# scttfrdmn/bwa-mem2-arm

Measured on AMD Instinct MI355X. Metric: M seed-extensions/sec (150 bp, band=100) at 1/2/4/8 MI355X vs CPU, higher is better.
Workload: dtype int16; 1 GPU; C2: 1000000 SeqPairs/GPU resident in HBM, 150 bp query / 300 bp ref, band w=100, cell_bits=16, h0 U[19,100]; pairs_per_gpu=1000000, parallelism=shard1 (independent pairs), distinct_gpus=1

## Files before the change

### bwa-mem2-arm_amd/csrc/bsw_pc.hip

```cpp
#include <hip/hip_runtime.h>
#include <stdint.h>
#include <stdlib.h>
#include <limits.h>
#include <utility>
#include "bsw_kernels.h"
#include "bsw_wave.h"

namespace bsw {

constexpr int kPcChunkDw = 17;
#ifndef BSW_PC_EXP_HALFHEAD
#define BSW_PC_EXP_HALFHEAD 0
#endif
#ifdef BSW_PC_STATS
__device__ unsigned long long g_pc_stats[13];
constexpr int kPcTimesMax = 1 << 16;
__device__ unsigned long long g_pc_times[kPcTimesMax][4];
#endif

struct PcRow {
    uint64_t enter;
    uint64_t fast;
    uint64_t left;
};

__device__ __forceinline__ uint64_t gbits(int lo, int n)
{
    uint64_t m;
    asm("s_bfm_b64 %0, %1, %2" : "=s"(m)
        : "s"(__builtin_amdgcn_readfirstlane(min(n, 63))), "s"(__builtin_amdgcn_readfirstlane(lo)));
    return m;
}

__device__ __forceinline__ uint32_t pack2(int v) { return ((uint32_t)v & 0xffffu) * 0x10001u; }

#define PC_SDWA(op, d, a, b, sel) \
    op "_sdwa " d ", " a ", " b " dst_sel:DWORD dst_unused:UNUSED_PAD src0_sel:DWORD src1_sel:" sel "\n\t"

#define PC_PH1_(X, EOUT, ESUB)                                                          \
    "v_pk_min_i16 %[s" X "], %[s" X "], %[h" X "]\n\t"                                      \
    "v_pk_add_u16 %[s" X "], %[s" X "], %[h" X "]\n\t"                                      \
    "v_pk_sub_i16 %[t" X "], %[s" X "], %[oe2]\n\t"                                         \
    "v_pk_max_i16 %[s" X "], %[s" X "], %[e" X "]\n\t"                                      \
    ESUB                                                                                     \
    "v_pk_max_i16 " EOUT ", " EOUT ", %[t" X "]\n\t"
#define PC_PH1(X, EOUT) PC_PH1_(X, EOUT, "v_pk_sub_i16 " EOUT ", %[e" X "], %[ed2]\n\t")
#define PC_PH1B(X, EOUT) PC_PH1_(X, EOUT, "v_pk_sub_u16 " EOUT ", %[e" X "], %[ed2] clamp\n\t")

#define PC_SCORES                                                                        \
    "v_perm_b32 %[y], %[phi], %[plo], %[q]\n\t"                                              \
    "v_pk_lshlrev_b16 %[sa], 8, %[y] op_sel_hi:[0,1]\n\t"                                    \
    "v_pk_ashrrev_i16 %[sa], 8, %[sa] op_sel_hi:[0,1]\n\t"                                   \
    "v_pk_ashrrev_i16 %[sb], 8, %[y] op_sel_hi:[0,1]\n\t"

#define PC_CELL(C, X, W)                                                                 \
    PC_SDWA("v_max_i32", C, "%[f]", "sext(%[s" X "])", W)                                    \
    "v_subrev_u32_e64 %[f], %[ed], %[f] clamp\n\t"                                           \
    PC_SDWA("v_max_i32", "%[f]", "%[f]", "sext(%[t" X "])", W)

#define PC_RESET(HP, RJ)                                                                 \
    "v_cmp_ne_u32_e32 vcc, " RJ ", %[begv]\n\t"                                              \
    "v_cndmask_b32_e32 " HP ", 0, " HP ", vcc\n\t"                                           \
    "v_cndmask_b32_e32 %[f], 0, %[f], vcc\n\t"
#define PC_MCELL(C, HP, X, W, J)                                                         \
    PC_CELL(C, X, W)                                                                         \
    "v_cmp_lt_i32_e32 vcc, " J ", %[endv]\n\t"                                               \
    "v_cndmask_b32_e32 " C ", " HP ", " C ", vcc\n\t"

#define PC_MWRITE(X, KEYSRC, LEFT)                                                       \
    "v_pk_sub_i16 %[y], %[jj" X "], %[endw]\n\t"                                             \
    "v_pk_ashrrev_i16 %[y], 15, %[y] op_sel_hi:[0,1]\n\t"                                    \
    "v_bfi_b32 %[h" X "], %[y], %[p" X "], %[h" X "]\n\t"                                    \
    "v_bfi_b32 %[e" X "], %[y], 0, %[e" X "]\n\t"                                            \
    KEYSRC                                                                                   \
    "v_and_b32_e32 %[p" X "], %[p" X "], %[y]\n\t"                                           \
    "v_pk_sub_i16 %[y], %[jj" X "], %[endm1w]\n\t"                                           \
    "v_pk_ashrrev_i16 %[y], 15, %[y] op_sel_hi:[0,1]\n\t"                                    \
    "v_bfi_b32 %[e" X "], %[y], %[x" X "], %[e" X "]\n\t"                                    \
    LEFT                                                                                     \
    "v_pk_max_u16 %[key], %[key], %[p" X "]\n\t"
#define PC_LEFTMASK(X)                                                                   \
    "v_pk_sub_i16 %[y], %[begm2w], %[jj" X "]\n\t"                                           \
    "v_pk_ashrrev_i16 %[y], 15, %[y] op_sel_hi:[0,1]\n\t"                                    \
    "v_and_b32_e32 %[p" X "], %[p" X "], %[y]\n\t"

#define PC_MASKED(CH0, CH1, CH2, CH3, KA, KB, LA, LB) PC_MASKED_(PC_PH1, CH0, CH1, CH2, CH3, KA, KB, LA, LB)
#define PC_MASKED_(PH, CH0, CH1, CH2, CH3, KA, KB, LA, LB)                               \
    PH("a", "%[xa]") PH("b", "%[xb]")                                                        \
    CH0 CH1                                                                                  \
    "v_lshl_or_b32 %[pa], %[c0], 16, %[h1]\n\t"                                              \
    CH2 CH3                                                                                  \
    "v_lshl_or_b32 %[pb], %[c2], 16, %[c1]\n\t"                                              \
    PC_MWRITE("a", KA, LA) PC_MWRITE("b", KB, LB)

#ifdef BSW_PC_STATS
#define PC_CNT(k) "v_add_u32_e32 %[ct" #k "], 1, %[ct" #k "]\n\t"
#define PC_CNT_OPS , [ct0] "+v"(ctr[0]), [ct1] "+v"(ctr[1]), [ct2] "+v"(ctr[2]), [ct3] "+v"(ctr[3])
#else
#define PC_CNT(k)
#define PC_CNT_OPS
#endif

#define PC_FAST_CHAIN                                                                    \
    PC_FAST_CHAIN_("v_alignbyte_b32 %[ha], %[pa], %[h1], 2\n\t", "v_alignbyte_b32 %[hb], %[h1], %[pa], 2\n\t")
#define PC_FAST_CHAIN_(A1, A2) PC_FAST_CHAIN__(A1, A2, "%[h1]")
#define PC_FAST_CHAIN__(A1, A2, H1O)                                                     \
    "v_pk_sub_u16 %[fp], %[f], %[e0e] op_sel_hi:[0,1] clamp\n\t"                            \
    "v_pk_max_i16 %[fp], %[fp], %[ta] op_sel_hi:[1,0]\n\t"                                  \
    "v_pk_max_i16 %[pa], %[fp], %[sa]\n\t"                                                  \
    "v_pk_sub_u16 %[fp], %[fp], %[ee2] op_sel:[1,0] clamp\n\t"                              \
    "v_pk_sub_i16 %[y], %[ta], %[e0e] op_sel:[1,0]\n\t"                                     \
    "v_pk_max_i16 %[fp], %[fp], %[y]\n\t"                                                   \
    A1                                                                                       \
    "v_pk_max_i16 %[fp], %[fp], %[tb] op_sel_hi:[1,0]\n\t"                                  \
    "v_pk_max_i16 " H1O ", %[fp], %[sb]\n\t"                                                \
    "v_sub_u32_sdwa %[f], %[fp], %[ed] clamp dst_sel:DWORD dst_unused:UNUSED_PAD src0_sel:WORD_1 src1_sel:DWORD\n\t" \
    A2                                                                                       \
    PC_SDWA("v_max_i32", "%[f]", "%[f]", "sext(%[tb])", "WORD_1")

#ifndef BSW_PC_RIGHT_EDGE
#define BSW_PC_RIGHT_EDGE 1
#endif
#define PC_REDGE(PH, KA, KB)                                                             \
    PH("a", "%[xa]") PH("b", "%[xb]")                                                        \
    PC_FAST_CHAIN__("v_alignbyte_b32 %[c0], %[pa], %[h1], 2\n\t",                            \
                    "v_alignbyte_b32 %[pb], %[c1], %[pa], 2\n\t", "%[c1]")                   \
    KA KB                                                                                    \
    "v_pk_sub_i16 %[sa], %[jja], %[endw]\n\t"                                                \
    "v_pk_sub_i16 %[sb], %[jjb], %[endw]\n\t"                                                \
    "v_pk_sub_i16 %[tb], %[jjb], %[endm1w]\n\t"                                              \
    "v_pk_ashrrev_i16 %[sa], 15, %[sa] op_sel_hi:[0,1]\n\t"                                  \
    "v_pk_ashrrev_i16 %[sb], 15, %[sb] op_sel_hi:[0,1]\n\t"                                  \
    "v_pk_ashrrev_i16 %[tb], 15, %[tb] op_sel_hi:[0,1]\n\t"                                  \
    "v_alignbyte_b32 %[ta], %[sb], %[sa], 2\n\t"                                             \
    "v_bfi_b32 %[h1], %[sa], %[c0], %[h1]\n\t"                                               \
    "v_bfi_b32 %[ha], %[sa], %[c0], %[ha]\n\t"                                               \
    "v_and_b32_e32 %[xa], %[xa], %[ta]\n\t"                                                  \
    "v_bfi_b32 %[h1], %[ta], %[pa], %[h1]\n\t"                                               \
    "v_bfi_b32 %[ea], %[sa], %[xa], %[ea]\n\t"                                               \
    "v_and_b32_e32 %[fp], %[fp], %[sa]\n\t"                                                  \
    "v_bfi_b32 %[h1], %[sb], %[pb], %[h1]\n\t"                                               \
    "v_bfi_b32 %[hb], %[sb], %[pb], %[hb]\n\t"                                               \
    "v_and_b32_e32 %[xb], %[xb], %[tb]\n\t"                                                  \
    "v_bfi_b32 %[h1], %[tb], %[c1], %[h1]\n\t"                                               \
    "v_bfi_b32 %[eb], %[sb], %[xb], %[eb]\n\t"                                               \
    "v_and_b32_e32 %[c2], %[c2], %[sb]\n\t"                                                  \
    "v_pk_max_u16 %[key], %[key], %[fp]\n\t"                                                 \
    "v_pk_max_u16 %[key], %[key], %[c2]\n\t"
#if BSW_PC_RIGHT_EDGE
#define PC_RBODY(PH, KA_M, KB_M, KA_R, KB_R) PC_REDGE(PH, KA_R, KB_R)
#else
#define PC_RBODY(PH, KA_M, KB_M, KA_R, KB_R)                                             \
    "v_lshrrev_b32_e32 %[h1], 16, %[h1]\n\t"                                                 \
    PC_MASKED_(PH, PC_MCELL("%[c0]", "%[h1]", "a", "WORD_0", "%[j0]"),                       \
                   PC_MCELL("%[c1]", "%[c0]", "a", "WORD_1", "%[j1]"),                       \
                   PC_MCELL("%[c2]", "%[c1]", "b", "WORD_0", "%[j2]"),                       \
                   PC_MCELL("%[h1]", "%[c2]", "b", "WORD_1", "%[j3]"), KA_M, KB_M, "", "")   \
    "v_lshlrev_b32_e32 %[h1], 16, %[h1]\n\t"
#endif
#define PC_LBODY(PH, KA_M, KB_M)                                                         \
    "v_lshrrev_b32_e32 %[h1], 16, %[h1]\n\t"          \
    PC_MASKED_(PH, PC_RESET("%[h1]", "%[r0]") PC_MCELL("%[c0]", "%[h1]", "a", "WORD_0", "%[j0]"), \
                   PC_RESET("%[c0]", "%[j1]") PC_MCELL("%[c1]", "%[c0]", "a", "WORD_1", "%[j1]"), \
                   PC_RESET("%[c1]", "%[j2]") PC_MCELL("%[c2]", "%[c1]", "b", "WORD_0", "%[j2]"), \
                   PC_RESET("%[c2]", "%[j3]") PC_MCELL("%[h1]", "%[c2]", "b", "WORD_1", "%[j3]"), \
                   KA_M, KB_M, PC_LEFTMASK("a"), PC_LEFTMASK("b"))                           \
    "v_lshlrev_b32_e32 %[h1], 16, %[h1]\n\t"

// ... 221 lines not shown
constexpr int kPcSeg = BSW_PC_SEG;
template <int QMAX> constexpr int pc_seg_len() { return QMAX <= 64 ? QMAX / 4 : kPcSeg; }
template <int QMAX, bool BY, int S, int... K>
__device__ __forceinline__ void pc_seg(std::integer_sequence<int, K...>, uint32_t (&hh)[(BY ? QMAX / 4 : QMAX / 2)],
                                       uint32_t (&ee)[(BY ? QMAX / 4 : QMAX / 2)], const uint32_t (&qs)[QMAX / 4], uint32_t plo,
                                       uint32_t phi, int &f, int &h1, uint32_t &key, uint32_t oe2, uint32_t ed2,
                                       int ed, const PcRow &r, uint32_t endw, uint32_t endm1w, uint32_t begm2w,
                                       int endv, int begv, const PcbSel &bs, uint32_t (&ctr)[4])
{
    constexpr int kSeg = sizeof...(K);
    constexpr uint64_t kSegMask = ((1ull << kSeg) - 1) << (kSeg * S);
    if (kSeg == QMAX / 4 || (r.enter & kSegMask))
        (pc_group_if<QMAX, BY, kSeg * S + K>(hh, ee, qs, plo, phi, f, h1, key, oe2, ed2, ed, r, endw, endm1w,
                                               begm2w, endv, begv, bs, ctr), ...);
}

template <int QMAX, bool BY, int... S>
__device__ __forceinline__ void pc_row(std::integer_sequence<int, S...>, uint32_t (&hh)[(BY ? QMAX / 4 : QMAX / 2)],
                                       uint32_t (&ee)[(BY ? QMAX / 4 : QMAX / 2)], const uint32_t (&qs)[QMAX / 4],
                                       uint32_t plo, uint32_t phi, int &f, int &h1, uint32_t &key,
                                       uint32_t oe2, uint32_t ed2, int ed, const PcRow &r,
                                       uint32_t endw, uint32_t endm1w, uint32_t begm2w, int endv,
                                       int begv, const PcbSel &bs, uint32_t (&ctr)[4])
{
    (pc_seg<QMAX, BY, S>(std::make_integer_sequence<int, pc_seg_len<QMAX>()>{}, hh, ee, qs, plo, phi, f, h1, key, oe2,
                         ed2, ed, r, endw, endm1w, begm2w, endv, begv, bs, ctr), ...);
}

template <int K>
__device__ __forceinline__ void pc_lastpos_reg(uint32_t hv, uint32_t endp1w, uint32_t &lp)
{
    constexpr uint32_t SC = (uint32_t)(2 * K) | ((uint32_t)(2 * K + 1) << 16);
    uint32_t c, m;
    asm volatile(
        "v_pk_min_u16 %[c], %[h], 1 op_sel_hi:[1,0]\n\t"
        "v_pk_mul_lo_u16 %[c], %[c], %[sc]\n\t"
        "v_pk_sub_i16 %[m], %[sc], %[e1]\n\t"
        "v_pk_ashrrev_i16 %[m], 15, %[m] op_sel_hi:[0,1]\n\t"
        "v_and_b32_e32 %[c], %[c], %[m]\n\t"
        "v_pk_max_u16 %[lp], %[lp], %[c]\n\t"
        : [lp] "+v"(lp), [c] "=&v"(c), [m] "=&v"(m)
        : [h] "v"(hv), [sc] "s"(SC), [e1] "v"(endp1w));
}

template <int QMAX, bool BY, int GG>
__device__ __forceinline__ bool pc_lastpos_group(const uint32_t (&hh)[(BY ? QMAX / 4 : QMAX / 2)], uint32_t endp1w,
                                                 bool pending, uint32_t &lp, int gstart)
{
    if (GG > gstart) return pending;
    if (__ballot(pending) == 0) return false;
    if constexpr (BY) {
        pc_lastpos_reg<2 * GG + 1>(__builtin_amdgcn_perm(hh[GG], hh[GG], kSelHi), endp1w, lp);
        pc_lastpos_reg<2 * GG>(__builtin_amdgcn_perm(hh[GG], hh[GG], kSelLo), endp1w, lp);
    } else {
        if constexpr (2 * GG + 1 < QMAX / 2) pc_lastpos_reg<2 * GG + 1>(hh[2 * GG + 1], endp1w, lp);
        pc_lastpos_reg<2 * GG>(hh[2 * GG], endp1w, lp);
    }
    return pending & (lp == 0u);
}

template <int QMAX, bool BY, int... G>
__device__ __forceinline__ int pc_lastpos(std::integer_sequence<int, G...>, const uint32_t (&hh)[(BY ? QMAX / 4 : QMAX / 2)],
                                          int end, bool need, int gstart)
{
    bool pending = need;
    uint32_t lp = 0;
    const uint32_t endp1w = pack2(end + 1);
    ((pending = pc_lastpos_group<QMAX, BY, QMAX / 4 - 1 - G>(hh, endp1w, pending, lp, gstart)), ...);
    return (int)max(lp & 0xffffu, lp >> 16);
}

#ifndef BSW_PC_EARLY_STOP
#define BSW_PC_EARLY_STOP 1
#endif
#ifndef BSW_PC_EARLY_SCAN
#define BSW_PC_EARLY_SCAN 1
#endif
#ifndef BSW_PC_SCAN_PHASE
#define BSW_PC_SCAN_PHASE 3
#endif

template <int K>
__device__ __forceinline__ void pc_ub_reg(uint32_t hv, uint32_t qw, uint32_t begw, uint32_t &ub)
{
    constexpr uint32_t SC = (uint32_t)(2 * K) | ((uint32_t)(2 * K + 1) << 16);
    uint32_t c, m;
    asm volatile(
        "v_pk_sub_i16 %[c], %[qw], %[sc]\n\t"
        "v_pk_ashrrev_i16 %[m], 15, %[c] op_sel_hi:[0,1]\n\t"
        "v_pk_add_u16 %[c], %[c], %[h]\n\t"
        "v_bfi_b32 %[c], %[m], 0, %[c]\n\t"
        "v_pk_sub_i16 %[m], %[bg], %[sc]\n\t"
        "v_pk_ashrrev_i16 %[m], 15, %[m] op_sel_hi:[0,1]\n\t"
        "v_and_b32_e32 %[c], %[c], %[m]\n\t"
        "v_pk_max_u16 %[ub], %[ub], %[c]\n\t"
        : [ub] "+v"(ub), [c] "=&v"(c), [m] "=&v"(m)
        : [h] "v"(hv), [qw] "v"(qw), [sc] "s"(SC), [bg] "v"(begw));
}

template <int QMAX, bool BY, int GG>
__device__ __forceinline__ void pc_ub_group(const uint32_t (&hh)[(BY ? QMAX / 4 : QMAX / 2)], uint32_t qw,
                                            uint32_t begw, uint32_t &ub, uint64_t enter)
{
    if (!((enter >> GG) & 1)) return;
    if constexpr (BY) {
        pc_ub_reg<2 * GG + 1>(__builtin_amdgcn_perm(hh[GG], hh[GG], kSelHi), qw, begw, ub);
        pc_ub_reg<2 * GG>(__builtin_amdgcn_perm(hh[GG], hh[GG], kSelLo), qw, begw, ub);
    } else {
        pc_ub_reg<2 * GG + 1>(hh[2 * GG + 1], qw, begw, ub);
        pc_ub_reg<2 * GG>(hh[2 * GG], qw, begw, ub);
    }
}

template <int QMAX, bool BY, int... G>
__device__ __forceinline__ int pc_ubscan(std::integer_sequence<int, G...>, const uint32_t (&hh)[(BY ? QMAX / 4 : QMAX / 2)],
                                         int qlen, int beg, uint64_t enter)
{
    uint32_t ub = 0;
    const uint32_t qw = pack2(qlen), begw = pack2(beg);
    (pc_ub_group<QMAX, BY, QMAX / 4 - 1 - G>(hh, qw, begw, ub, enter), ...);
    return (int)max(ub & 0xffffu, ub >> 16);
}

#ifndef BSW_PC_LEFT_SKIP
#define BSW_PC_LEFT_SKIP 1
#endif
#ifndef BSW_PC_SKIP_MASK
#define BSW_PC_SKIP_MASK 3
#endif
#ifndef BSW_PC_SKIP_ROW
#define BSW_PC_SKIP_ROW 1
#endif
#ifndef BSW_PC_SKIP_QMIN
#define BSW_PC_SKIP_QMIN 96
#endif
template <int QMAX> constexpr bool pc_left_skip() { return BSW_PC_LEFT_SKIP && QMAX >= BSW_PC_SKIP_QMIN; }

#ifndef BSW_PC_LEFT_PRUNE
#define BSW_PC_LEFT_PRUNE 1
#endif
#ifndef BSW_PC_PRUNE_QMIN
#define BSW_PC_PRUNE_QMIN 128
#endif
template <int QMAX, bool BY> constexpr bool pc_left_prune()
{
    return BSW_PC_LEFT_PRUNE && !BY && pc_left_skip<QMAX>() && QMAX >= BSW_PC_PRUNE_QMIN;
}
#ifndef BSW_PC_PRUNE_BRANCH
#define BSW_PC_PRUNE_BRANCH 1
#endif
constexpr int kPcPruned = 1 << 8;
template <bool PRUNE> __device__ __forceinline__ int pc_gz_of(int gz) { return PRUNE ? (gz & (kPcPruned - 1)) : gz; }

template <int K>
__device__ __forceinline__ void pc_pb_reg(uint32_t v, uint32_t gw, uint32_t bw, uint32_t &ub)
{
    constexpr uint32_t SC = (uint32_t)(2 * K) | ((uint32_t)(2 * K + 1) << 16);
    uint32_t c, m;
    asm volatile(
        "v_pk_sub_i16 %[c], %[gw], %[sc]\n\t"
        "v_pk_min_u16 %[m], %[v], 1 op_sel_hi:[1,0]\n\t"
        "v_pk_mul_lo_u16 %[c], %[c], %[m]\n\t"
        "v_pk_add_u16 %[c], %[c], %[v]\n\t"
        "v_pk_sub_i16 %[m], %[bw], %[sc]\n\t"
        "v_pk_ashrrev_i16 %[m], 15, %[m] op_sel_hi:[0,1]\n\t"
        "v_and_b32_e32 %[c], %[c], %[m]\n\t"
        "v_pk_max_u16 %[ub], %[ub], %[c]\n\t"
        : [ub] "+v"(ub), [c] "=&v"(c), [m] "=&v"(m)
        : [v] "v"(v), [gw] "v"(gw), [sc] "s"(SC), [bw] "v"(bw));
}

__device__ __forceinline__ uint32_t pc_pos2(uint32_t e)
{
    uint32_t r;
    asm volatile("v_pk_max_i16 %0, %1, 0" : "=v"(r) : "v"(e));
    return r;
}

struct PcPrune {
    bool pre;
    int qlen, beg, gsc;
    uint32_t npr;
};

template <int QMAX, bool BY, bool PRUNE, int G>
__device__ __forceinline__ void pc_gz_group(uint32_t (&hh)[(BY ? QMAX / 4 : QMAX / 2)],
                                            uint32_t (&ee)[(BY ? QMAX / 4 : QMAX / 2)], bool live, int &gz, PcPrune &pp)
{
    if constexpr (G < QMAX / 4) {
        if (pc_gz_of<PRUNE>(gz) != G) return;
        uint32_t z;
        if constexpr (BY) {
            asm volatile("v_or_b32_e32 %0, %1, %2" : "=v"(z) : "v"(hh[G]), "v"(ee[G]));
        } else {
            uint32_t t;
            asm volatile("v_pk_max_i16 %0, %2, 0\n\t"
                         "v_pk_max_i16 %1, %3, 0\n\t"
                         "v_or3_b32 %0, %0, %1, %4\n\t"
                         "v_or_b32_e32 %0, %0, %5"
                         : "=&v"(z), "=&v"(t)
                         : "v"(ee[2 * G]), "v"(ee[2 * G + 1]), "v"(hh[2 * G]), "v"(hh[2 * G + 1]));
        }
        if (__ballot(live && z != 0u) == 0) {
            gz = PRUNE ? gz + 1 : G + 1;
        } else if constexpr (PRUNE) {
            if (!pp.pre) return;
            uint32_t ub = 0;
            const uint32_t qw = pack2(pp.qlen), qm1w = pack2(pp.qlen - 1);
            const uint32_t bgw = pack2(pp.beg), bgm1w = pack2(pp.beg - 1);
            static_assert(!BY, "the byte planes are compiled without the prune");
            pc_pb_reg<2 * G + 1>(hh[2 * G + 1], qw, bgw, ub);
            pc_pb_reg<2 * G>(hh[2 * G], qw, bgw, ub);
            pc_pb_reg<2 * G + 1>(pc_pos2(ee[2 * G + 1]), qm1w, bgm1w, ub);
            pc_pb_reg<2 * G>(pc_pos2(ee[2 * G]), qm1w, bgm1w, ub);
            const int u = (int)max(ub & 0xffffu, ub >> 16);
            if (__ballot(live && u >= pp.gsc) == 0) {
                hh[2 * G] = 0u; hh[2 * G + 1] = 0u; ee[2 * G] = 0u; ee[2 * G + 1] = 0u;
                gz = (G + 1) | kPcPruned;
#ifdef BSW_PC_STATS
                pp.npr += 1;
#endif
            }
        }
    }
}

template <int QMAX, bool BY, bool PRUNE, int S, int... K>
__device__ __forceinline__ void pc_gz_seg(std::integer_sequence<int, K...>, uint32_t (&hh)[(BY ? QMAX / 4 : QMAX / 2)],
                                          uint32_t (&ee)[(BY ? QMAX / 4 : QMAX / 2)], bool live, int &gz, PcPrune &pp)
{
    if ((pc_gz_of<PRUNE>(gz) >> 3) != S) return;
    (pc_gz_group<QMAX, BY, PRUNE, 8 * S + K>(hh, ee, live, gz, pp), ...);
}

template <int QMAX, bool BY, bool PRUNE, int... S>
__device__ __forceinline__ void pc_gz_refresh(std::integer_sequence<int, S...>, uint32_t (&hh)[(BY ? QMAX / 4 : QMAX / 2)],
                                              uint32_t (&ee)[(BY ? QMAX / 4 : QMAX / 2)], bool live, int &gz, PcPrune &pp)
{
    (pc_gz_seg<QMAX, BY, PRUNE, S>(std::make_integer_sequence<int, 8>{}, hh, ee, live, gz, pp), ...);
}

template <int QMAX, int WPB, bool BY, bool REDO>
__global__ __launch_bounds__(64 * WPB, BY ? 3 : 2) void pc_kernel(const KParams kp, const int32_t w,
                                                    SeqPair *__restrict__ pairs,
                                                    const int32_t *__restrict__ order,
                                                    const int32_t n_in,
                                                    const uint8_t *__restrict__ ref,
                                                    const uint8_t *__restrict__ qer,
                                                    int32_t *__restrict__ err,
                                                    int32_t *__restrict__ redo,
                                                    int32_t *__restrict__ rcnt)
{
    constexpr bool PRUNE = !REDO && pc_left_prune<QMAX, BY>();
    constexpr int NG = QMAX / 4;
    constexpr int CDW = kPcChunkDw;
#ifdef BSW_PC_STATS
    const unsigned long long t_wave0 = wall_clock64();
#endif
    __shared__ uint32_t s_tgt[WPB][2][CDW][64];
    __shared__ uint2 s_prof[8];
    int32_t n = n_in;
    if constexpr (REDO) {
        n = min(n, *rcnt);
        if ((int)(blockIdx.x * blockDim.x) >= n) return;
    }
    if (threadIdx.x < 8) s_prof[threadIdx.x] = make_uint2(kp.prof[threadIdx.x][0], kp.prof[threadIdx.x][1]);
    __syncthreads();
    const int gid = blockIdx.x * blockDim.x + threadIdx.x;
    bool valid = gid < n;
    const int idx = valid ? (order ? order[gid] : gid) : 0;
    SeqPair *sp = pairs + idx;
    int idr = 0, idq = 0, tlen = 0, qlen = 0, h0 = 0;
    if (valid) {
        idr = sp->idr; idq = sp->idq; tlen = sp->len1; qlen = sp->len2; h0 = sp->h0;
        if (qlen >= QMAX || qlen < 0 || tlen < 0 || h0 < 0 || h0 + min(qlen, tlen) > 255 || idr < 0 || idq < 0) {
            atomicOr(err, 1);
            valid = false;
        }
    }
    uint32_t qs[NG];
    {
        uint32_t wv[NG + 1];
        const uintptr_t qa = (uintptr_t)(qer + idq);
        const uint32_t *wp = (const uint32_t *)(qa & ~(uintptr_t)3);
        const int sh = (int)(qa & 3);
        const int nw = (valid && qlen > 0) ? (sh + qlen + 3) >> 2 : 0;
        if (nw > 0) {
#pragma unroll
            for (int g = 0; g <= NG; ++g) wv[g] = wp[min(g, nw - 1)];
        } else {
#pragma unroll
            for (int g = 0; g <= NG; ++g) wv[g] = 0;
        }
#pragma unroll
        for (int g = 0; g < NG; ++g) {
            const uint32_t c = __builtin_amdgcn_alignbyte(wv[g + 1], wv[g], sh);
            qs[g] = __builtin_amdgcn_perm(c, c, 0x03010200u);
        }
    }
    constexpr int NP = (BY ? QMAX / 4 : QMAX / 2);
    uint32_t hh[NP], ee[NP];
    {
        const int oe_ins = kp.o_ins + kp.e_ins;
        if constexpr (BY) {
            __builtin_amdgcn_sched_barrier(0);
#pragma unroll
            for (int k = 0; k < NP; ++k) {
                uint32_t v[4];
#pragma unroll
                for (int t = 0; t < 4; ++t) {
                    const int j = 4 * k + t;
                    v[t] = (j == 0) ? (uint32_t)h0 : (j <= qlen) ? (uint32_t)max(h0 - oe_ins - (j - 1) * kp.e_ins, 0) : 0u;
                }
                hh[k] = v[0] | (v[1] << 8) | (v[2] << 16) | (v[3] << 24);
                asm volatile("" : "+v"(hh[k]));
                ee[k] = 0u;
            }
        } else {
#pragma unroll
            for (int k = 0; k < NP; ++k) {
                const int j0 = 2 * k, j1 = 2 * k + 1;
                const uint32_t a = (j0 == 0) ? (uint32_t)h0
                                 : (j0 <= qlen) ? (uint32_t)max(h0 - oe_ins - (j0 - 1) * kp.e_ins, 0) : 0u;
                const uint32_t b = (j1 <= qlen) ? (uint32_t)max(h0 - oe_ins - (j1 - 1) * kp.e_ins, 0) : 0u;
                hh[k] = a | (b << 16);
                ee[k] = 0u;
            }
        }
    }
    int wl = w;
    {
        const int ni = qlen * kp.maxsc + kp.end_bonus - kp.o_ins;
        const int nd = qlen * kp.maxsc + kp.end_bonus - kp.o_del;
        wl = min(wl, max((ni + kp.e_ins) / kp.e_ins, 1));
        wl = min(wl, max((nd + kp.e_del) / kp.e_del, 1));
    }
    int best = h0, best_i = -1, best_j = -1, max_ie = -1, gsc = -1, moff = 0, endc = qlen;
    bool alive = valid && tlen > 0;
    if (!valid) sp = nullptr;
    asm volatile("" : "+v"(sp));
    const uint8_t *tp = ref + idr;
    const int tsh = (int)((uintptr_t)tp & 3);
    const uint32_t *twp = (const uint32_t *)(tp - tsh);
    const int tlast = max((tsh + tlen - 1) >> 2, 0);
    const int wv = threadIdx.x >> 6, ln = threadIdx.x & 63;
    auto issue_chunk = [&](int ch) {
        uint32_t *dst = &s_tgt[wv][ch & 1][0][0];
#pragma unroll
        for (int k = 0; k < CDW; ++k)
            __builtin_amdgcn_global_load_lds((gptr_t)(twp + min(16 * ch + k, tlast)),
                                             (lptr_t)(dst + 64 * k), 4, 0, 0);
    };
    if (alive) { issue_chunk(0); issue_chunk(1); }
    uint32_t tcur = 0;
    const int wl_max = wave_max(alive ? wl : -1);
    const int wl_min = wave_min(alive ? wl : INT_MAX);
    const uint32_t oe2 = (uint32_t)(kp.o_del + kp.e_del) * 0x10001u;
    const uint32_t ed2 = (uint32_t)kp.e_del * 0x10001u;
    uint32_t ctr[4] = {0, 0, 0, 0};
    PcbSel bs{BY ? kSelKa : 0x06010400u, BY ? kSelKb : 0x06030402u};
    if constexpr (BY || (BSW_PC_JKEY && QMAX >= 128)) asm volatile("" : "+v"(bs.ka), "+v"(bs.kb));
#ifdef BSW_PC_STATS
    uint32_t nrows = 0, nlast = 0, nue = 0;
    uint32_t nscan = 0, nstop_s = 0, nstop_c = 0;
    (void)nscan; (void)nstop_s; (void)nstop_c;
#endif

#if BSW_PC_EXP_HALFHEAD
    int emax = 0, emin = 0;
    PcRow r{0, 0, 0};
#endif
    int gz = 0;
    (void)gz;
    PcPrune pp{false, 0, 0, 0, 0u};
    for (int i = 0;; ++i) {
        const bool act = alive && i < tlen;
        alive = act;
        if (__ballot(act) == 0) break;
        if ((i & 3) == 0) {
            if ((i & 63) == 0) {
                __builtin_amdgcn_s_waitcnt(0x0F70);
                __builtin_amdgcn_sched_barrier(0);
            }
            const int k = (i >> 2) & 15;
            const uint32_t la = (uint32_t)(uintptr_t)(lptr_t)&s_tgt[wv][(i >> 6) & 1][k][ln];
            uint2 d;
            asm volatile("ds_read2st64_b32 %0, %1 offset1:1\n\ts_waitcnt lgkmcnt(0)"
                         : "=v"(d) : "v"(la) : "memory");
            tcur = __builtin_amdgcn_alignbyte(d.y, d.x, tsh);
            if ((i & 63) == 0) {
                __builtin_amdgcn_sched_barrier(0);
                if (i > 0 && act) issue_chunk((i >> 6) + 1);
            }
        }
        const uint32_t tcode = (tcur >> (8 * (i & 3))) & 0xffu;
        const uint2 pr = s_prof[min(tcode, 7u)];
        __builtin_amdgcn_sched_barrier(0);
        const int beg = max(0, i - wl);
        const int end = min(min(endc, i + wl + 1), qlen);
        endc = end;
#if BSW_PC_EXP_HALFHEAD
        if (i & 1) goto row_body;
#else
        int emax, emin;
        PcRow r;
#endif
        wave_maxmin_bc(act ? end : -1, act ? end : INT_MAX, emax, emin);
        {
            const int ulo = __builtin_amdgcn_readfirstlane(max(0, i - wl_max));
            const int uhi = __builtin_amdgcn_readfirstlane(emax);
            const int flo = __builtin_amdgcn_readfirstlane(max(0, i - wl_min));
            const int fhi = __builtin_amdgcn_readfirstlane(emin);
            const int glo = ulo >> 2;
            const int gsp = max((min(uhi, QMAX - 1) >> 2) - glo, -1);
            const int gfa = (ulo == flo && (flo & 3) == 0) ? (flo >> 2) : (flo >> 2) + 1;
            const int gfn = max((fhi >> 2) - gfa, 0);
            const int gln = (flo >> 2) - glo;
            r.enter = gbits(glo, gsp + 1);
            r.fast = gbits(gfa, gfn);
            r.left = gbits(glo, gln + 1);
            if constexpr (pc_left_skip<QMAX>()) {
                const uint64_t keep = ~0ull << pc_gz_of<PRUNE>(gz);
                r.enter &= keep;
                r.fast &= keep;
            }
        }
#if BSW_PC_EXP_HALFHEAD
    row_body:
#endif
        {
            int h1 = (int)((uint32_t)max(h0 - (kp.o_del + kp.e_del * (i + 1)), 0) << 16) & -(int)(beg == 0);
            int f = 0;
            uint32_t key = 0;
            const uint32_t endw = pack2(end);
            const uint32_t endm1w = pack2(end - 1);
            const uint32_t begm2w = pack2(beg - 2);
            __builtin_amdgcn_s_setprio(0);
            pc_row<QMAX, BY>(std::make_integer_sequence<int, (NG + pc_seg_len<QMAX>() - 1) / pc_seg_len<QMAX>()>{}, hh, ee,
                             qs, pr.x, pr.y, f, h1, key, oe2, ed2, kp.e_del, r, endw, endm1w, begm2w, end, beg, bs,
                             ctr);
            __builtin_amdgcn_s_setprio(2);
            h1 = (int)((uint32_t)h1 >> 16);
            const uint32_t k32 = max(key & 0xffffu, key >> 16);
            const int m = (int)(k32 >> 8), mj = (int)(k32 & 0xffu);
            {
                const bool atq = act && end == qlen;
                max_ie = (atq && !(gsc > h1)) ? i : max_ie;
                gsc = atq ? max(gsc, h1) : gsc;
            }
            {
                const int di = i - best_i, dj = mj - best_j;
                const int dz = (di > dj) ? best - m - (int)__umul24((unsigned)(di - dj), (unsigned)kp.e_del)
                                         : best - m - (int)__umul24((unsigned)(dj - di), (unsigned)kp.e_ins);
                const bool better = act && m > best;
                const bool zdropped = kp.zdrop > 0 && dz > kp.zdrop;
                alive = act && m > 0 && (better || !zdropped);
                moff = better ? max(moff, abs(mj - i)) : moff;
                best_i = better ? i : best_i;
                best_j = better ? mj : best_j;
                best = better ? m : best;
                if constexpr (PRUNE) {
#if BSW_PC_PRUNE_BRANCH
                    if (gz & kPcPruned)
#endif
                    {
                        const bool rd = (gz & kPcPruned) != 0 &&
                                        ((act && !better && m > 0 && kp.zdrop > 0 && best - m > kp.zdrop) ||
                                         (alive && h1 == 0));
                        alive = alive && !rd;
                        sp = (SeqPair *)((uintptr_t)sp | (uintptr_t)rd);
                    }
                }
            }
#if BSW_PC_EARLY_STOP
            {
                int gq, gt, gm;
                asm volatile("v_sub_u32_e32 %0, %3, %4\n\t"
                             "v_subrev_u32_e32 %1, %5, %6\n\t"
                             "v_sub_u32_e32 %2, %3, %7"
                             : "=&v"(gq), "=&v"(gt), "=&v"(gm)
                             : "v"(qlen), "v"(beg), "s"(i), "v"(tlen), "v"(mj));
                const bool edge = end == qlen && gq < qlen;
                const int ubs = m - 1 + min(gq, gt);
                const bool stop = edge && ubs <= best && ubs < gsc;
#ifdef BSW_PC_STATS
                nstop_s += alive && stop;
#endif
                alive = alive && !stop;
#if BSW_PC_EARLY_SCAN
                const int ubm = m - 1 + gm;
                const bool want = QMAX > 64 && alive && edge && ubm <= best && ubm < gsc;
                if (QMAX > 64 && (i & BSW_PC_SCAN_PHASE) == BSW_PC_SCAN_PHASE && __ballot(want)) {
                    const int ubc = pc_ubscan<QMAX, BY>(std::make_integer_sequence<int, NG>{}, hh, gq + beg, beg, r.enter);
                    const bool stopc = want && ubc <= best && ubc < gsc;
#ifdef BSW_PC_STATS
                    nscan += 1;
                    nstop_c += stopc;
#endif
                    alive = alive && !stopc;
                }
#endif
            }
#endif
            if constexpr (pc_left_skip<QMAX>()) {
                if ((i & BSW_PC_SKIP_MASK) == BSW_PC_SKIP_ROW) {
                    if constexpr (PRUNE) {
                        pp.pre = i > wl_max && __ballot(alive && !(end == qlen && gsc > 0)) == 0;
                        asm volatile("v_mov_b32_e32 %0, %1" : "=v"(pp.qlen) : "v"(qlen));
                        pp.beg = beg; pp.gsc = gsc;
                    }
                    pc_gz_refresh<QMAX, BY, PRUNE>(std::make_integer_sequence<int, (NG + 7) / 8>{}, hh, ee, alive, gz,
                                                   pp);
                }
            }
#ifdef BSW_PC_STATS
            nrows += act;
            nue += act && (emax == emin);
#endif
            {
                const bool need = alive && h1 == 0;
                int lp1 = end;
                if (__ballot(need)) {
#ifdef BSW_PC_STATS
                    nlast += 1;
#endif
                    const int lp = pc_lastpos<QMAX, BY>(std::make_integer_sequence<int, NG>{}, hh, end, need,
                                                        emax >> 2);
                    lp1 = need ? lp : end;
                }
                endc = alive ? min(lp1 + 2, qlen) : endc;
            }
        }
    }
#ifdef BSW_PC_STATS
    {
        const unsigned rows = (unsigned)wave_max((int)nrows);
        const unsigned nl = (unsigned)wave_max((int)nlast);
        const unsigned nu = (unsigned)wave_max((int)nue);
        const unsigned ns = (unsigned)wave_max((int)nscan);
        const unsigned rs = (unsigned)__popcll(__ballot(nstop_s != 0));
        const unsigned rc = (unsigned)__popcll(__ballot(nstop_c != 0));
        unsigned cmax[4];
        for (int k = 0; k < 4; ++k) cmax[k] = (unsigned)wave_max((int)ctr[k]);
        if ((threadIdx.x & 63) == 0) {
            atomicAdd(&g_pc_stats[0], (unsigned long long)rows);
            for (int k = 0; k < 4; ++k) atomicAdd(&g_pc_stats[1 + k], (unsigned long long)cmax[k]);
            atomicAdd(&g_pc_stats[5], (unsigned long long)nl);
            atomicAdd(&g_pc_stats[6], 1ull);
            atomicAdd(&g_pc_stats[7], (unsigned long long)nu);
            atomicAdd(&g_pc_stats[8], (unsigned long long)ns);
            atomicAdd(&g_pc_stats[9], (unsigned long long)rs);
            atomicAdd(&g_pc_stats[10], (unsigned long long)rc);
        }
        const unsigned wid = blockIdx.x * WPB + (threadIdx.x >> 6);
        if ((threadIdx.x & 63) == 0 && wid < (unsigned)kPcTimesMax) {
            unsigned xcc, hw;
            asm volatile("s_getreg_b32 %0, hwreg(HW_REG_XCC_ID)" : "=s"(xcc));
            asm volatile("s_getreg_b32 %0, hwreg(HW_REG_HW_ID)" : "=s"(hw));
            g_pc_times[wid][0] = t_wave0;
            g_pc_times[wid][1] = wall_clock64();
            g_pc_times[wid][2] = ((unsigned long long)xcc << 32) | hw;
            g_pc_times[wid][3] = rows;
        }
    }
#endif
    if constexpr (PRUNE) {
        const bool rd = ((uintptr_t)sp & 1u) != 0;
        const unsigned long long rb = __ballot(rd);
        if (rb) {
            int base = 0;
            if (ln == __ffsll((long long)rb) - 1) base = atomicAdd(rcnt, (int)__popcll(rb));
            base = __shfl(base, __ffsll((long long)rb) - 1);
            if (rd) {
                const unsigned g = blockIdx.x * blockDim.x + threadIdx.x;
                redo[base + (int)__popcll(rb & ((1ull << ln) - 1ull))] = order ? order[g] : (int)g;
            }
        }
#ifdef BSW_PC_STATS
        if (ln == 0) {
            atomicAdd(&g_pc_stats[11], (unsigned long long)pp.npr);
            atomicAdd(&g_pc_stats[12], (unsigned long long)__popcll(rb));
        }
#endif
        if (rd) sp = nullptr;
    }
    if (sp) {
        sp->score = best;
        sp->tle = best_i + 1;
        sp->gtle = max_ie + 1;
        sp->qle = best_j + 1;
        sp->gscore = gsc;
        sp->max_off = moff;
    }
}

#ifdef BSW_PC_STATS
extern "C" int bsw_pc_stats(unsigned long long *out, int reset)
{
    if (hipMemcpyFromSymbol(out, HIP_SYMBOL(g_pc_stats), 13 * sizeof(unsigned long long)) != hipSuccess) return -5;
    if (reset) {
        unsigned long long z[13] = {0, 0, 0, 0, 0, 0, 0, 0, 0, 0, 0, 0, 0};
        if (hipMemcpyToSymbol(HIP_SYMBOL(g_pc_stats), z, sizeof(z)) != hipSuccess) return -5;
    }
    return 0;
}
extern "C" int bsw_pc_times(unsigned long long *out, int n)
{
    n = n < kPcTimesMax ? n : kPcTimesMax;
    if (hipMemcpyFromSymbol(out, HIP_SYMBOL(g_pc_times), (size_t)n * 32) != hipSuccess) return -5;
    return n;
}
#endif

template <int QMAX>
static void launch_pc_q(const KParams &kp, int32_t w, SeqPair *pairs, const int32_t *order, int32_t n,
                        const uint8_t *ref, const uint8_t *qer, int32_t *err, int32_t *redo, int32_t *rcnt,
                        hipStream_t s)
{
    const unsigned grid = (unsigned)((n + 63) / 64);
    if (kp.kern8 == 2)
        hipLaunchKernelGGL((pc_kernel<QMAX, 1, true, false>), dim3(grid), dim3(64), 0, s, kp, w, pairs, order, n,
                           ref, qer, err, redo, rcnt);
    else
        hipLaunchKernelGGL((pc_kernel<QMAX, 1, false, false>), dim3(grid), dim3(64), 0, s, kp, w, pairs, order,
                           n, ref, qer, err, redo, rcnt);
    if constexpr (pc_left_prune<QMAX, false>()) {
        constexpr int kRedoWpb = 4;
        const unsigned rgrid = (unsigned)((n + 64 * kRedoWpb - 1) / (64 * kRedoWpb));
        if (kp.kern8 != 2)
            hipLaunchKernelGGL((pc_kernel<QMAX, kRedoWpb, false, true>), dim3(rgrid), dim3(64 * kRedoWpb), 0, s, kp, w,
                               pairs, redo, n, ref, qer, err, nullptr, rcnt);
    }
}

hipError_t launch_pc_kernel(int qmax, const KParams &kp, int32_t w, SeqPair *pairs,
                            const int32_t *order, int32_t n, const uint8_t *ref,
                            const uint8_t *qer, int32_t *err, int32_t *redo, int32_t *rcnt, hipStream_t s)
{
    if (n <= 0) return hipSuccess;
    if (!redo || !rcnt) return hipErrorInvalidValue;
    switch (qmax) {
    case 32: launch_pc_q<32>(kp, w, pairs, order, n, ref, qer, err, redo, rcnt, s); break;
    case 64: launch_pc_q<64>(kp, w, pairs, order, n, ref, qer, err, redo, rcnt, s); break;
    case 96: launch_pc_q<96>(kp, w, pairs, order, n, ref, qer, err, redo, rcnt, s); break;
    case 128: launch_pc_q<128>(kp, w, pairs, order, n, ref, qer, err, redo, rcnt, s); break;
    case 160: launch_pc_q<160>(kp, w, pairs, order, n, ref, qer, err, redo, rcnt, s); break;
    default: return hipErrorInvalidValue;
    }
    return hipGetLastError();
}

}
```

Baseline: 189.2 M seed-extensions/s.

## Add speculative right-side band pruning with redo fallback in banded SW kernel

Adds a right-prune mode that walks column groups from the right and zeroes the H/E registers of any group whose best possible reachable score cannot come within a margin of the current best. The band end is then capped so later rows skip those groups. Lanes whose result might have been affected by clipping are marked for the existing redo pass, with a threshold packed into the high bits of the SeqPair pointer. This cuts per-row work on the right edge of the band, at the cost of extra ballots and walk overhead, more redo launches, and reliance on pointer high bits being free.

Result: faster. 193.7 M seed-extensions/s (median of 6 runs) (+2.4%).

```diff
diff --git a/bwa-mem2-arm_amd/csrc/bsw_pc.hip b/bwa-mem2-arm_amd/csrc/bsw_pc.hip
--- a/bwa-mem2-arm_amd/csrc/bsw_pc.hip
+++ b/bwa-mem2-arm_amd/csrc/bsw_pc.hip
@@ -13,7 +13,7 @@
 #define BSW_PC_EXP_HALFHEAD 0
 #endif
 #ifdef BSW_PC_STATS
-__device__ unsigned long long g_pc_stats[13];
+__device__ unsigned long long g_pc_stats[19];
 constexpr int kPcTimesMax = 1 << 16;
 __device__ unsigned long long g_pc_times[kPcTimesMax][4];
 #endif
@@ -541,6 +541,44 @@
 constexpr int kPcPruned = 1 << 8;
 template <bool PRUNE> __device__ __forceinline__ int pc_gz_of(int gz) { return PRUNE ? (gz & (kPcPruned - 1)) : gz; }
 
+#ifndef BSW_PC_RIGHT_PRUNE
+#define BSW_PC_RIGHT_PRUNE 1
+#endif
+#ifndef BSW_PC_RP_MARGIN
+#define BSW_PC_RP_MARGIN 20
+#endif
+#ifndef BSW_PC_RP_SLACK
+#define BSW_PC_RP_SLACK 12
+#endif
+#ifndef BSW_PC_RP_SLACK2
+#define BSW_PC_RP_SLACK2 11
+#endif
+#ifndef BSW_PC_RP_K
+#define BSW_PC_RP_K 16
+#endif
+#ifndef BSW_PC_RP_WALK_MASK
+#define BSW_PC_RP_WALK_MASK 15
+#endif
+#ifndef BSW_PC_RP_RWIN
+#define BSW_PC_RP_RWIN 4
+#endif
+#ifndef BSW_PC_RP_ROW0
+#define BSW_PC_RP_ROW0 25
+#endif
+template <int QMAX, bool BY> constexpr bool pc_right_prune() { return BSW_PC_RIGHT_PRUNE && pc_left_prune<QMAX, BY>(); }
+constexpr int kPcPShift = 54;
+constexpr uintptr_t kPcClipped = (uintptr_t)1 << 53;
+constexpr uint32_t kPcClipHi = (uint32_t)(kPcClipped >> 32), kPcLowHi = (1u << (kPcPShift - 32)) - 1u;
+__device__ __forceinline__ uint32_t pc_sp_hi(const SeqPair *sp) { return (uint32_t)((uintptr_t)sp >> 32); }
+__device__ __forceinline__ SeqPair *pc_sp_set(const SeqPair *sp, uint32_t hi, bool rd)
+{
+    return (SeqPair *)(((uintptr_t)hi << 32) | (uintptr_t)(uint32_t)(uintptr_t)sp | (uintptr_t)rd);
+}
+__device__ __forceinline__ uint32_t pc_rp_raise(uint32_t hi, int t)
+{
+    return max(hi, ((uint32_t)(max(t, 0) + 1) << (kPcPShift - 32)) | (hi & kPcLowHi));
+}
+
 template <int K>
 __device__ __forceinline__ void pc_pb_reg(uint32_t v, uint32_t gw, uint32_t bw, uint32_t &ub)
 {
@@ -629,6 +667,43 @@
     (pc_gz_seg<QMAX, BY, PRUNE, S>(std::make_integer_sequence<int, 8>{}, hh, ee, live, gz, pp), ...);
 }
 
+template <int QMAX, int G>
+__device__ __forceinline__ void pc_rp_group(uint32_t (&hh)[QMAX / 2], uint32_t (&ee)[QMAX / 2], bool live, int gzv,
+                                            int &cap4, int qlen, int t, uint32_t &nev)
+{
+    if (cap4 != 4 * G + 4 || G < gzv + 2) return;
+    uint32_t ub = 0;
+    const uint32_t qw = pack2(qlen), qm1w = pack2(qlen - 1), allw = 0xffffffffu;
+    pc_pb_reg<2 * G + 1>(hh[2 * G + 1], qw, allw, ub);
+    pc_pb_reg<2 * G>(hh[2 * G], qw, allw, ub);
+    pc_pb_reg<2 * G + 1>(pc_pos2(ee[2 * G + 1]), qm1w, allw, ub);
+    pc_pb_reg<2 * G>(pc_pos2(ee[2 * G]), qm1w, allw, ub);
+    const int u = max((int)max(ub & 0xffffu, ub >> 16), 1 + qlen - 4 * G);
+    if (__ballot(live && u + BSW_PC_RP_SLACK >= t) == 0) {
+        hh[2 * G] = 0u; hh[2 * G + 1] = 0u; ee[2 * G] = 0u; ee[2 * G + 1] = 0u;
+        cap4 = 4 * G;
+        nev += 1;
+    }
+}
+
+template <int QMAX, int S, int... K>
+__device__ __forceinline__ void pc_rp_seg(std::integer_sequence<int, K...>, uint32_t (&hh)[QMAX / 2],
+                                          uint32_t (&ee)[QMAX / 2], bool live, int gzv, int &cap4, int qlen, int t,
+                                          uint32_t &nev)
+{
+    if (((cap4 - 4) >> 5) < S) return;
+    (pc_rp_group<QMAX, 8 * S + 7 - K>(hh, ee, live, gzv, cap4, qlen, t, nev), ...);
+}
+
+template <int QMAX, int... S>
+__device__ __forceinline__ void pc_rp_walk(std::integer_sequence<int, S...>, uint32_t (&hh)[QMAX / 2],
+                                           uint32_t (&ee)[QMAX / 2], bool live, int gzv, int &cap4, int qlen, int t,
+                                           uint32_t &nev)
+{
+    constexpr int NS = sizeof...(S);
+    (pc_rp_seg<QMAX, NS - 1 - S>(std::make_integer_sequence<int, 8>{}, hh, ee, live, gzv, cap4, qlen, t, nev), ...);
+}
+
 template <int QMAX, int WPB, bool BY, bool REDO>
 __global__ __launch_bounds__(64 * WPB, BY ? 3 : 2) void pc_kernel(const KParams kp, const int32_t w,
                                                     SeqPair *__restrict__ pairs,
@@ -641,6 +716,7 @@
                                                     int32_t *__restrict__ rcnt)
 {
     constexpr bool PRUNE = !REDO && pc_left_prune<QMAX, BY>();
+    constexpr bool RP = !REDO && pc_right_prune<QMAX, BY>();
     constexpr int NG = QMAX / 4;
     constexpr int CDW = kPcChunkDw;
 #ifdef BSW_PC_STATS
@@ -665,6 +741,12 @@
         if (qlen >= QMAX || qlen < 0 || tlen < 0 || h0 < 0 || h0 + min(qlen, tlen) > 255 || idr < 0 || idq < 0) {
             atomicOr(err, 1);
             valid = false;
+        }
+        if constexpr (!REDO && pc_right_prune<QMAX, BY>()) {
+            if ((uintptr_t)sp >> 53) {
+                atomicOr(err, 1);
+                valid = false;
+            }
         }
     }
     uint32_t qs[NG];
@@ -762,6 +844,14 @@
     int gz = 0;
     (void)gz;
     PcPrune pp{false, 0, 0, 0, 0u};
+    int cap4 = QMAX;
+    bool rmark = false;
+    uint32_t nrev = 0;
+    (void)cap4; (void)rmark; (void)nrev;
+#ifdef BSW_PC_STATS
+    uint32_t nrcap = 0, nrret = 0, rcause = 0;
+    (void)nrcap; (void)nrret; (void)rcause;
+#endif
     for (int i = 0;; ++i) {
         const bool act = alive && i < tlen;
         alive = act;
@@ -786,7 +876,15 @@
         const uint2 pr = s_prof[min(tcode, 7u)];
         __builtin_amdgcn_sched_barrier(0);
         const int beg = max(0, i - wl);
-        const int end = min(min(endc, i + wl + 1), qlen);
+        int endcl = min(min(endc, i + wl + 1), qlen);
+#ifdef BSW_PC_STATS
+        if constexpr (RP) {
+            const int eu = wave_max(act ? min(i + wl + 1, qlen) : -1), ec = wave_max(act ? min(endcl, cap4) : -1);
+            if (cap4 < QMAX && ec >= 0) nrcap += (uint32_t)max((min(eu, QMAX - 1) >> 2) - (min(ec, QMAX - 1) >> 2), 0);
+        }
+#endif
+        if constexpr (RP) endcl = min(endcl, cap4);
+        const int end = endcl;
         endc = end;
 #if BSW_PC_EXP_HALFHEAD
         if (i & 1) goto row_body;
@@ -850,14 +948,31 @@
                 best = better ? m : best;
                 if constexpr (PRUNE) {
 #if BSW_PC_PRUNE_BRANCH
-                    if (gz & kPcPruned)
+                    if ((gz & kPcPruned) || (RP && rmark))
 #endif
                     {
-                        const bool rd = (gz & kPcPruned) != 0 &&
+                        const bool rd = ((gz & kPcPruned) != 0 || (RP && rmark)) &&
                                         ((act && !better && m > 0 && kp.zdrop > 0 && best - m > kp.zdrop) ||
-                                         (alive && h1 == 0));
+                                         ((gz & kPcPruned) != 0 && alive && h1 == 0));
                         alive = alive && !rd;
                         sp = (SeqPair *)((uintptr_t)sp | (uintptr_t)rd);
+#ifdef BSW_PC_STATS
+                        rcause = (rd && !rcause) ? 2u : rcause;
+#endif
+                    }
+                }
+                if constexpr (RP) {
+                    if (rmark) {
+                        const int t = best - BSW_PC_RP_MARGIN, phi = h1 + (qlen - end);
+                        uint32_t hi = pc_sp_hi(sp);
+                        const bool cl = act && end < qlen && (end == cap4 || (hi & kPcClipHi) != 0);
+                        const bool rdc = cl && h1 > 0 && phi >= t;
+                        hi = cl ? pc_rp_raise(hi | kPcClipHi, t) : hi;
+                        sp = pc_sp_set(sp, hi, rdc);
+                        alive = alive && !rdc;
+#ifdef BSW_PC_STATS
+                        rcause = (rdc && !rcause) ? 1u : rcause;
+#endif
                     }
                 }
             }
@@ -900,6 +1015,35 @@
                     }
                     pc_gz_refresh<QMAX, BY, PRUNE>(std::make_integer_sequence<int, (NG + 7) / 8>{}, hh, ee, alive, gz,
                                                    pp);
+                    if constexpr (RP) {
+                        if (__ballot(alive && !(i >= BSW_PC_RP_ROW0 && i - best_i <= BSW_PC_RP_K))) {
+                            if (cap4 < QMAX) {
+                                cap4 += 4;
+#ifdef BSW_PC_STATS
+                                nrret += 1;
+#endif
+                            }
+                        } else if ((!rmark || (i & BSW_PC_RP_WALK_MASK) == (BSW_PC_SKIP_ROW & BSW_PC_RP_WALK_MASK)) &&
+                                   __ballot(alive)) {
+                            int ql;
+                            asm volatile("v_mov_b32_e32 %0, %1" : "=v"(ql) : "v"(qlen));
+                            const uint32_t nev0 = nrev;
+                            pc_rp_walk<QMAX>(std::make_integer_sequence<int, NG / 8>{}, hh, ee, alive,
+                                             pc_gz_of<PRUNE>(gz), cap4, ql, best - BSW_PC_RP_MARGIN, nrev);
+                            if (nrev != nev0) {
+                                rmark = true;
+                                sp = pc_sp_set(sp, alive ? pc_rp_raise(pc_sp_hi(sp), best - BSW_PC_RP_MARGIN) : pc_sp_hi(sp), false);
+                            }
+                        }
+                        if (rmark && cap4 < QMAX &&
+                            __ballot(alive && end < qlen && end + BSW_PC_RP_RWIN >= cap4 &&
+                                     h1 + (qlen - end) + BSW_PC_RP_SLACK2 >= best - BSW_PC_RP_MARGIN)) {
+                            cap4 += 4;
+#ifdef BSW_PC_STATS
+                            nrret += 1;
+#endif
+                        }
+                    }
                 }
             }
 #ifdef BSW_PC_STATS
@@ -954,6 +1098,14 @@
     }
 #endif
     if constexpr (PRUNE) {
+        if constexpr (RP) {
+            const int pf = (int)((uintptr_t)sp >> kPcPShift);
+            const bool rdf = pf != 0 && gsc < pf - 1;
+#ifdef BSW_PC_STATS
+            rcause = (rdf && !((uintptr_t)sp & 1u)) ? 3u : rcause;
+#endif
+            sp = (SeqPair *)((((uintptr_t)sp) | (uintptr_t)rdf) & (kPcClipped - 1));
+        }
         const bool rd = ((uintptr_t)sp & 1u) != 0;
         const unsigned long long rb = __ballot(rd);
         if (rb) {
@@ -969,6 +1121,13 @@
         if (ln == 0) {
             atomicAdd(&g_pc_stats[11], (unsigned long long)pp.npr);
             atomicAdd(&g_pc_stats[12], (unsigned long long)__popcll(rb));
+            atomicAdd(&g_pc_stats[13], (unsigned long long)nrev);
+            atomicAdd(&g_pc_stats[14], (unsigned long long)nrcap);
+            atomicAdd(&g_pc_stats[15], (unsigned long long)nrret);
+        }
+        for (unsigned c = 1; c <= 3; ++c) {
+            const unsigned nc = (unsigned)__popcll(__ballot(rd && rcause == c));
+            if (ln == 0 && nc) atomicAdd(&g_pc_stats[15 + c], (unsigned long long)nc);
         }
 #endif
         if (rd) sp = nullptr;
@@ -986,9 +1145,9 @@
 #ifdef BSW_PC_STATS
 extern "C" int bsw_pc_stats(unsigned long long *out, int reset)
 {
-    if (hipMemcpyFromSymbol(out, HIP_SYMBOL(g_pc_stats), 13 * sizeof(unsigned long long)) != hipSuccess) return -5;
+    if (hipMemcpyFromSymbol(out, HIP_SYMBOL(g_pc_stats), 19 * sizeof(unsigned long long)) != hipSuccess) return -5;
     if (reset) {
-        unsigned long long z[13] = {0, 0, 0, 0, 0, 0, 0, 0, 0, 0, 0, 0, 0};
+        unsigned long long z[19] = {0};
         if (hipMemcpyToSymbol(HIP_SYMBOL(g_pc_stats), z, sizeof(z)) != hipSuccess) return -5;
     }
     return 0;
```
